# cbg-ethz/metMHN

Measured on AMD Instinct MI355X. Metric: full-cohort log-lik+grad evals/sec at n=20 events; kronvec HBM GB/s, higher is better.
Workload: dtype f64

## Files before the change

### metmhn_amd/csrc/wlayout.h

```cpp
#pragma once
#include <hip/hip_runtime.h>
#include "desc.h"

namespace mmhn {

__host__ __device__ inline int popc32(uint32_t v) {
#ifdef __HIP_DEVICE_COMPILE__
  return __popc(v);
#else
  return __builtin_popcount(v);
#endif
}
__host__ __device__ inline uint32_t pext32(uint32_t x, uint32_t mask) {
  uint32_t out = 0, pos = 0;
  while (mask) {
    const uint32_t low = mask & (0u - mask);
    if (x & low) out |= 1u << pos;
    ++pos;
    mask ^= low;
  }
  return out;
}
__host__ __device__ inline uint32_t pdep32(uint32_t v, uint32_t mask) {
  uint32_t out = 0;
  while (mask) {
    const uint32_t low = mask & (0u - mask);
    if (v & 1u) out |= low;
    v >>= 1;
    mask ^= low;
  }
  return out;
}

constexpr int WLB = 6, WWB = 4, WTB = WLB + WWB;
constexpr int WROWS = 1 << WTB;
constexpr int WMAXB = 20;

template <typename T> struct WCfg;
#ifndef MMHN_WHB
#define MMHN_WHB 2
#endif
#ifndef MMHN_WNXT_D
#define MMHN_WNXT_D (7 - MMHN_WHB)
#endif
template <> struct WCfg<double> {
  static constexpr int RB = 2, HB = MMHN_WHB, KC = 9, KR = 15, KE = 9, PAD = 2, NXT = MMHN_WNXT_D;
  static constexpr bool FACT = false, REV = true, ON = true;
};
#ifndef MMHN_WF32
#define MMHN_WF32 1
#endif
template <> struct WCfg<float> {
  static constexpr int RB = 3, HB = 2, KC = 12, KR = 18, KE = 12, PAD = 4, NXT = 9;
  static constexpr bool FACT = true, REV = false, ON = MMHN_WF32 != 0;
};

struct WDesc {
  int prob;
  int kR, kC, majP;
  int nXc, nXr;
  uint32_t rowmask, colmask;
  uint32_t pairRowC;
  uint32_t loneRowC;
  int8_t rb[WMAXB];
  int8_t cb[WMAXB];
  int8_t prt[WMAXB];
};

struct W6 {
  uint8_t rank[64], order[64], off[8], cnt[8];
};
constexpr W6 make_w6() {
  W6 t{};
  int pos = 0;
  for (int m = 0; m <= 6; ++m) {
    t.off[m] = (uint8_t)pos;
    int r = 0;
    for (int l = 0; l < 64; ++l) {
      int pc = 0;
      for (int b = 0; b < 6; ++b) pc += (l >> b) & 1;
      if (pc == m) { t.rank[l] = (uint8_t)r++; t.order[pos++] = (uint8_t)l; }
    }
    t.cnt[m] = (uint8_t)r;
  }
  t.off[7] = 64; t.cnt[7] = 0;
  return t;
}
__host__ __device__ inline uint32_t wrho(uint32_t w, uint32_t l) {
  constexpr W6 t = make_w6();
  const int m = popc32(l);
  return 16u * t.off[m] + w * t.cnt[m] + t.rank[l];
}
__host__ __device__ inline uint32_t wrho_inv(uint32_t r) {
  constexpr W6 t = make_w6();
  int m = 0;
  while (r >= 16u * t.off[m + 1]) ++m;
  const uint32_t q = r - 16u * t.off[m];
  return ((q / t.cnt[m]) << 6) | t.order[t.off[m] + q % t.cnt[m]];
}
template <typename T>
__host__ __device__ inline long long wpos(uint32_t Sigma, uint32_t beta, uint32_t rho, uint32_t c) {
  return ((((long long)((Sigma << WCfg<T>::HB) | beta) << WTB) + rho) << WCfg<T>::RB) + c;
}
template <typename T>
__host__ __device__ inline long long wpos_nat(const WDesc& w, uint32_t x) {
  constexpr int RB = WCfg<T>::RB, HB = WCfg<T>::HB;
  const uint32_t S = pext32(x, w.rowmask), Tc = pext32(x, w.colmask);
  const uint32_t Sigma = (Tc >> (RB + HB)) | ((S >> WTB) << w.nXc);
  return wpos<T>(Sigma, (Tc >> RB) & ((1u << HB) - 1u), wrho((S >> WLB) & ((1u << WWB) - 1u), S & 63u), Tc & ((1u << RB) - 1u));
}

template <typename T>
__host__ __device__ inline long long wpos_marg(const WDesc& w, int k, bool free_is_row, uint32_t f) {
  constexpr int RB = WCfg<T>::RB, HB = WCfg<T>::HB;
  const long long half = 1ll << (k - 1);
  if (free_is_row) {
    const uint32_t Sigma = ((1u << w.nXc) - 1u) | ((f >> WTB) << w.nXc);
    return half + wpos<T>(Sigma, (1u << HB) - 1u, wrho((f >> WLB) & ((1u << WWB) - 1u), f & 63u), (1u << RB) - 1u);
  }
  const uint32_t Sigma = (f >> (RB + HB)) | (((1u << w.nXr) - 1u) << w.nXc);
  return half + wpos<T>(Sigma, (f >> RB) & ((1u << HB) - 1u), (uint32_t)WROWS - 1u, f & ((1u << RB) - 1u));
}

}
```

Measured before the change: 21.70.

## Reorder packed row layout by joint popcount of high and low bit groups

Changes the rho permutation of the 10-bit row index so rows are grouped first by the popcount of the 4 high bits and then by a custom order of the low 6-bit popcount classes, through a precomputed base table. The inverse mapping and the marginal position computation are updated to match, since the all-ones row is no longer at the end. The intent is for rows touched together by the kronvec sweeps to sit closer in memory, giving more contiguous HBM access. It adds table lookups and a more complex inverse that loops over classes.

New measurement: 22.08 (median of 6 runs). 1.8% higher.

```diff
diff --git a/metmhn_amd/csrc/wlayout.h b/metmhn_amd/csrc/wlayout.h
--- a/metmhn_amd/csrc/wlayout.h
+++ b/metmhn_amd/csrc/wlayout.h
@@ -69,6 +69,10 @@
 
 struct W6 {
   uint8_t rank[64], order[64], off[8], cnt[8];
+  uint8_t mseq[8];
+  uint8_t wseq[16], lamoff[6];
+  uint16_t lamrow[6];
+  uint16_t base[16][8];
 };
 constexpr W6 make_w6() {
   W6 t{};
@@ -84,19 +88,38 @@
     t.cnt[m] = (uint8_t)r;
   }
   t.off[7] = 64; t.cnt[7] = 0;
+  constexpr int mseq[7] = {0, 2, 1, 5, 3, 4, 6};
+  for (int i = 0; i < 7; ++i) t.mseq[i] = (uint8_t)mseq[i];
+  int row = 0, nw = 0;
+  for (int lam = 0; lam <= WWB; ++lam) {
+    t.lamoff[lam] = (uint8_t)nw;
+    t.lamrow[lam] = (uint16_t)row;
+    int first = nw;
+    for (int w = 0; w < (1 << WWB); ++w) {
+      int pc = 0;
+      for (int b = 0; b < WWB; ++b) pc += (w >> b) & 1;
+      if (pc == lam) t.wseq[nw++] = (uint8_t)w;
+    }
+    for (int i = 0; i < 7; ++i)
+      for (int j = first; j < nw; ++j) { t.base[t.wseq[j]][mseq[i]] = (uint16_t)row; row += t.cnt[mseq[i]]; }
+  }
+  t.lamoff[WWB + 1] = (uint8_t)nw; t.lamrow[WWB + 1] = (uint16_t)row;
   return t;
 }
 __host__ __device__ inline uint32_t wrho(uint32_t w, uint32_t l) {
   constexpr W6 t = make_w6();
-  const int m = popc32(l);
-  return 16u * t.off[m] + w * t.cnt[m] + t.rank[l];
+  return (uint32_t)t.base[w][popc32(l)] + t.rank[l];
 }
 __host__ __device__ inline uint32_t wrho_inv(uint32_t r) {
   constexpr W6 t = make_w6();
-  int m = 0;
-  while (r >= 16u * t.off[m + 1]) ++m;
-  const uint32_t q = r - 16u * t.off[m];
-  return ((q / t.cnt[m]) << 6) | t.order[t.off[m] + q % t.cnt[m]];
+  int lam = 0;
+  while (r >= t.lamrow[lam + 1]) ++lam;
+  const uint32_t nw = (uint32_t)(t.lamoff[lam + 1] - t.lamoff[lam]);
+  uint32_t q = r - t.lamrow[lam];
+  int i = 0;
+  while (q >= nw * t.cnt[t.mseq[i]]) { q -= nw * t.cnt[t.mseq[i]]; ++i; }
+  const int m = t.mseq[i];
+  return ((uint32_t)t.wseq[t.lamoff[lam] + q / t.cnt[m]] << 6) | t.order[t.off[m] + q % t.cnt[m]];
 }
 template <typename T>
 __host__ __device__ inline long long wpos(uint32_t Sigma, uint32_t beta, uint32_t rho, uint32_t c) {
@@ -119,7 +142,7 @@
     return half + wpos<T>(Sigma, (1u << HB) - 1u, wrho((f >> WLB) & ((1u << WWB) - 1u), f & 63u), (1u << RB) - 1u);
   }
   const uint32_t Sigma = (f >> (RB + HB)) | (((1u << w.nXr) - 1u) << w.nXc);
-  return half + wpos<T>(Sigma, (f >> RB) & ((1u << HB) - 1u), (uint32_t)WROWS - 1u, f & ((1u << RB) - 1u));
+  return half + wpos<T>(Sigma, (f >> RB) & ((1u << HB) - 1u), wrho((1u << WWB) - 1u, 63u), f & ((1u << RB) - 1u));
 }
 
 }
```
